# facebookresearch/any4

Hardware: AMD Instinct MI355X
Metric: any4 W4A16 GEMM achieved GB/s (m=1, n=k=4096, g=128) (higher is better)
Workload: dtype bf16

## Files before the change

any4_amd/csrc/tg_gemv.hip:

```cpp
#include "tg_common.cuh"
namespace {
#include "w4_helpers.cuh"
#include "w4_gemv.cuh"

#ifndef TG_GEMV_MF_MIN_M
#define TG_GEMV_MF_MIN_M 1
#endif
#ifndef TG_GEMV_MAX_TILES
#define TG_GEMV_MAX_TILES 16384
#endif
}

#if GEMV_TRACE
static TraceRing g_trace;
extern "C" TG_API void tg_dev_gemv_trace(unsigned long long* buf, int slots) { g_trace.set(buf, slots); }
#endif

int tgx::gemv(const GemmParams& p) {
  const int g0 = 1 << p.gshift;
#ifndef TG_GEMV_MF_MAX_M
#define TG_GEMV_MF_MAX_M 8
#endif
  const bool mf = p.m >= TG_GEMV_MF_MIN_M && p.m <= TG_GEMV_MF_MAX_M && (g0 == 128 || g0 == 256) && (p.k <= 4096 || p.m <= 4) && p.ksuper % 2 == 0;
  if (p.inner != 4 || p.qmx || (p.m > 4 && !mf) || p.x_tc || p.y_tc || p.batch != 1) return TG_PAIR_NA;
  if (p.ksuper * 64 != p.k || p.ntiles * 8 != p.wrows || p.ntiles > TG_GEMV_MAX_TILES) return TG_PAIR_NA;
  const int g = 1 << p.gshift;
  const int gps = g == 32 ? 2 : 1;
  GemvParams gp;
  copy_call(gp, p);
  gp.sg_shift = g <= 64 ? 0 : g == 128 ? 1 : 2;
  gp.trace = nullptr;
  gp.cm = (mf && p.m >= 6 && (p.k == 4096 || p.k == 2048)) ? 1 : 0;
  gp.unit = p.epilogue == TG_EPI_SWIGLU ? 2 : 1;
  if (p.ntiles % gp.unit != 0) return TG_PAIR_NA;
  const int units = p.ntiles / gp.unit;
  const int cus = plan_cu_count(p);
#ifndef TG_GEMV_WG2_MIN_BYTES
#define TG_GEMV_WG2_MIN_BYTES (48ll << 20)
#endif
  auto lds_two_per_cu = [&]() -> int64_t {
    const int tpw2 = ((units + 2 * cus - 1) / (2 * cus)) * gp.unit;
    const int64_t xs = (int64_t)p.m * (p.k / 4), xsmf = mf ? (int64_t)(p.k / 128) * 64 : 0;
    return 65536 + (p.qtype == TG_Q_ANY4_ROWWISE ? tpw2 * 8 * 32 : 0) + (int64_t)p.m * (p.k * 2 + (p.m > 1 ? 16 : 0)) + (xsmf > xs ? xsmf : xs) +
           2 * 8 * p.m * 32 * 4 + 8 * p.m * 4;
  };
  auto padded_tiles = [&](int n_wgs) -> int64_t {
    const int ub = units / n_wgs, ur = units % n_wgs;
    auto pad2 = [&](int u) -> int64_t { return (int64_t)((u * gp.unit + 1) / 2) * 2; };
    return ur * pad2(ub + 1) + (int64_t)(n_wgs - ur) * pad2(ub);
  };
#ifndef TG_GEMV_WG2_MIN_UNITS_PER_CU
#define TG_GEMV_WG2_MIN_UNITS_PER_CU 4
#endif
  const bool two_per_cu = (int64_t)p.wrows * p.k / 2 >= TG_GEMV_WG2_MIN_BYTES && units >= TG_GEMV_WG2_MIN_UNITS_PER_CU * cus && lds_two_per_cu() <= 80 * 1024 &&
                          padded_tiles(2 * cus) <= padded_tiles(cus);
  const int wgs = units < cus ? units : (two_per_cu ? 2 * cus : cus);
  gp.ubase = units / wgs;
  gp.urem = units % wgs;
  gp.uextra = 1;
#ifndef TG_GEMV_WG2_EXTRA
#define TG_GEMV_WG2_EXTRA 3
#endif
  if (TG_GEMV_WG2_EXTRA > 1 && two_per_cu && wgs == 2 * cus && units % cus == 0 && (units / cus) % 2 == 1 && units / cus > TG_GEMV_WG2_EXTRA) {
    gp.ubase = (units / cus - TG_GEMV_WG2_EXTRA) / 2;
    gp.urem = cus;
    gp.uextra = TG_GEMV_WG2_EXTRA;
  }
  gp.uh = 0;
  const int tpw = (gp.ubase + (gp.urem ? gp.uextra : 0)) * gp.unit;
#ifndef TG_GEMV_P_BIG
#define TG_GEMV_P_BIG 16
#endif
  gp.P = mf ? 16 : tpw <= 1 ? 8 : tpw <= 2 ? 16 : TG_GEMV_P_BIG;
  if (p.ksuper % 2 != 0) gp.P = 32;
  else if (p.ksuper % 4 != 0 && gp.P < 16) gp.P = 16;
  gp.p_shift = gp.P == 8 ? 3 : gp.P == 16 ? 4 : 5;
  const int tpp = gp.P / 8;
  const int passes = (tpw + tpp - 1) / tpp;
  const int SS = 32 / gp.P;
  gp.spw = ((p.ksuper + 7) / 8 + SS - 1) / SS * SS;
  gp.spp = gp.spw / SS;
  const int d = gp.spp <= 4 ? 4 : 8;
  gp.rounds = (gp.spp + d - 1) / d;
  gp.xcd4 = (gp.urem == 0 && wgs % 32 == 0) ? 1 : 0;
  if (p.k > 16384) return TG_PAIR_NA;
  gp.lds_lut = 65536;
  const bool stage_lut = p.qtype == TG_Q_ANY4_ROWWISE && passes > 1;
  gp.x_pitch = p.k * 2 + (p.m > 1 ? 16 : 0);
  gp.lds_x = gp.lds_lut + (stage_lut ? tpw * 8 * 32 : 0);
  gp.xs_pitch = p.k / 4;
  gp.lds_xs = gp.lds_x + p.m * gp.x_pitch;
  gp.lds_red = gp.lds_xs + (mf && (p.k / 128) * 64 > p.m * gp.xs_pitch ? (p.k / 128) * 64 : p.m * gp.xs_pitch);
  gp.lds_nrm = gp.lds_red + 2 * 8 * p.m * 32 * 4;
  const unsigned lds = (unsigned)gp.lds_nrm + (unsigned)(8 * p.m * 4);
  if (lds > 160u * 1024u) return TG_PAIR_NA;
  if (p.dry) return TG_PLAN_GEMV;
  const dim3 grid((unsigned)wgs, (unsigned)p.batch);
#if GEMV_TRACE
  gp.trace = g_trace.next();
#endif
  return pick_dt(p.dt, [&](auto DT_) {
    using DT = decltype(DT_);
    return pick<1, 2, 3, 4, 5, 6, 7, 8>(p.m, [&](auto M_) {
      return pick<1, 2>(gps, [&](auto GPS_) {
        return pick<4, 8>(d, [&](auto D_) {
          return pick<0, 1>(p.norm_w != nullptr, [&](auto NORM_) {
            return pick<0, 1>(mf, [&](auto MF_) {
              constexpr int M = decltype(M_)::value, GPS = decltype(GPS_)::value, D = decltype(D_)::value;
              constexpr bool NORM = decltype(NORM_)::value, MF = decltype(MF_)::value;
              if constexpr (MF ? (M < TG_GEMV_MF_MIN_M || GPS != 1 || (D == 8 && M > 4)) : M > 4) {
                return (int)TG_PAIR_NA;
              } else {
                return launch_lds_kernel<w4_gemv_kernel<DT, M, GPS, D, NORM, MF>>(grid, dim3(512), lds, p.st, gp, true);
              }
            });
          });
        });
      });
    });
  });
}
```

any4_amd/csrc/w4_gemv.cuh:

```cuda
#pragma once

struct GemvParams {
  const char* x;
  const char* w;
  const char* qinfo;
  const char* lut;
  char* y;
  const char* bias;
  const char* norm_w;
  int64_t stride_x, stride_w, stride_qinfo, stride_lut, stride_y, stride_bias;
  int64_t bias_row_stride;
  int32_t m, wrows, k;
  int32_t ntiles;
  int32_t ksuper;
  int32_t qtype;
  int32_t sg_shift;
  int32_t P, p_shift;
  int32_t unit;
  int32_t ubase, urem;
  int32_t uextra;
  int32_t uh;
  int32_t spw;
  int32_t spp;
  int32_t rounds;
  int32_t x_pitch, xs_pitch;
  int32_t lds_lut, lds_x, lds_xs, lds_red, lds_nrm;
  float norm_eps;
  int32_t epilogue;
  int32_t xcd4;
  int32_t cm;
  unsigned long long* trace;
};

template <typename DT, int M, int GPS, int D, bool NORM, bool MF = false>
__global__ void __launch_bounds__(512, 2) w4_gemv_kernel(const GemvParams p) {
  static_assert(!MF || GPS == 1, "matrix-core contraction: groups of at least two super-tiles");
#ifndef TG_GEMV_MF_ONES_MIN_M
#define TG_GEMV_MF_ONES_MIN_M 5
#endif
  constexpr bool MFS = MF && M >= TG_GEMV_MF_ONES_MIN_M;
  constexpr int NW = 8, NT = NW * 64;
  const int tid = threadIdx.x;
  const int lane = tid & 63;
  const int wave = __builtin_amdgcn_readfirstlane(tid >> 6);
  constexpr int b = 0;
  TG_TRACE_BEGIN();
  TG_STAMP(0);

  asm volatile("" ::"s"(p.x), "s"(p.w), "s"(p.qinfo), "s"(p.lut), "s"(p.y), "s"(p.bias), "s"(p.norm_w), "s"(p.stride_x), "s"(p.stride_w),
               "s"(p.stride_qinfo), "s"(p.stride_lut), "s"(p.stride_y), "s"(p.stride_bias), "s"(p.bias_row_stride));
  asm volatile("" ::"s"(p.m), "s"(p.wrows), "s"(p.k), "s"(p.ksuper), "s"(p.qtype), "s"(p.sg_shift), "s"(p.P), "s"(p.p_shift), "s"(p.unit),
               "s"(p.ubase), "s"(p.urem), "s"(p.spw), "s"(p.spp), "s"(p.rounds), "s"(p.x_pitch), "s"(p.xs_pitch), "s"(p.lds_lut),
               "s"(p.lds_x), "s"(p.lds_xs), "s"(p.lds_red), "s"(p.lds_nrm), "s"(p.norm_eps), "s"(p.epilogue), "s"(p.xcd4), "s"(p.cm), "s"(p.uextra), "s"(p.uh));
  TG_STAMP(6);

  int bx = blockIdx.x;
  if (p.xcd4) bx = (((bx >> 5) * 8 + (bx & 7)) << 2) + ((bx >> 3) & 3);
  int t0 = bx * p.ubase + min(bx, p.urem) * p.uextra, nu = p.ubase + (bx < p.urem ? p.uextra : 0);
  if (p.uh) {
    const int c = bx < p.urem ? bx : bx - p.urem;
    t0 += bx < p.urem ? min(c, p.uh) : p.uh - min(c, p.uh);
    nu += c < p.uh ? (bx < p.urem ? 1 : -1) : 0;
  }
  t0 *= p.unit;
  const int t1 = t0 + nu * p.unit;
  if (t0 >= t1) return;
  const int P = p.P, Pm = P - 1, tpp = P >> 3;
  const int passes = (t1 - t0 + tpp - 1) >> (p.p_shift - 3);
  const int row_l = lane & Pm;
  const int sub = lane >> p.p_shift;
  const int h = sub & 1, ss = sub >> 1;
  const int SS = 32 >> p.p_shift;
  const int s_begin = wave * p.spw;
  const int s_end = min(s_begin + p.spw, p.ksuper);
  const int spp = p.spp;
  const int rounds = p.rounds;

  const char* wb = p.w + (int64_t)b * p.stride_w;
  const char* qb = p.qinfo + (int64_t)b * p.stride_qinfo;
  const char* lb = p.lut + (int64_t)b * p.stride_lut;
  const char* xb = p.x + (int64_t)b * p.stride_x;

  struct Slot {
    u32x4 w;
    uint32_t q[GPS];
  };
  Slot ring[D];
  int ip = 0, ii = 0;
  uint32_t wlane, qlane;
  const uint32_t qrow_bytes = (uint32_t)p.wrows * 4u;
  auto pass_lane = [&](int pass) {
    const int tile = min(t0 + pass * tpp + (row_l >> 3), t1 - 1);
    wlane = (uint32_t)tile * (uint32_t)p.ksuper * 256u + (uint32_t)((row_l & 7) * 32 + h * 16 + ss * 256);
    qlane = (uint32_t)(tile * 8 + (row_l & 7)) * 4u + (uint32_t)(GPS == 1 ? (ss >> p.sg_shift) : 2 * ss) * qrow_bytes;
  };
  pass_lane(0);
  const int slots = rounds * D;
  const int su_max = p.ksuper - SS;
  auto issue = [&](Slot& sl) {
    const int su = min(s_begin + min(ii, spp - 1) * SS, su_max);
    sl.w = __builtin_nontemporal_load(reinterpret_cast<const u32x4*>(wb + (uint32_t)su * 256u + wlane));
    if constexpr (GPS == 1) {
      sl.q[0] = *reinterpret_cast<const uint32_t*>(qb + (uint32_t)(su >> p.sg_shift) * qrow_bytes + qlane);
    } else {
      sl.q[0] = *reinterpret_cast<const uint32_t*>(qb + (uint32_t)(2 * su) * qrow_bytes + qlane);
      sl.q[1] = *reinterpret_cast<const uint32_t*>(qb + (uint32_t)(2 * su + 1) * qrow_bytes + qlane);
    }
    if (++ii == slots) {
      ii = 0;
      if (ip + 1 < passes) pass_lane(++ip);
      else ii = slots - 1;
    }
  };

  const int npc = p.k >> 3;
  const int nch = p.k >> 5;
  const bool wide = npc > NT;
  uint32_t xd[M][16];
  uint32_t gwd[NORM ? 16 : 1];
  auto stage_load = [&](const char* base, uint32_t (&d)[16]) {
    if (!wide) {
      const int pc = min(tid, npc - 1);
      const char* src = base + (pc >> 2) * 64 + (pc & 3) * 4;
#pragma unroll
      for (int j = 0; j < 4; ++j) d[j] = *reinterpret_cast<const uint32_t*>(src + j * 16);
#pragma unroll
      for (int j = 4; j < 16; ++j) d[j] = 0u;
    } else {
      const u32x4* src = reinterpret_cast<const u32x4*>(base + min(tid, nch - 1) * 64);
#pragma unroll
      for (int j = 0; j < 4; ++j) {
        const u32x4 v = src[j];
        d[4 * j] = v[0]; d[4 * j + 1] = v[1]; d[4 * j + 2] = v[2]; d[4 * j + 3] = v[3];
      }
    }
  };
  bool cm = false;
  int cm_row = 0, cm_chunk = 0, cm_rpr = 1;
  if constexpr (M >= 5) {
    cm = p.cm != 0;
    cm_rpr = NT / nch;
    cm_row = tid / nch;
    cm_chunk = tid - cm_row * nch;
  }
  if (M >= 5 && cm) {
#pragma unroll
    for (int j = 0; j < M; ++j) {
      if (j * cm_rpr < M) {
        const int row = min(j * cm_rpr + cm_row, M - 1);
        const u32x4* src = reinterpret_cast<const u32x4*>(xb + (int64_t)row * p.k * 2 + cm_chunk * 64);
#pragma unroll
        for (int q = 0; q < 4; ++q) {
          const u32x4 v = src[q];
          xd[j][4 * q] = v[0]; xd[j][4 * q + 1] = v[1]; xd[j][4 * q + 2] = v[2]; xd[j][4 * q + 3] = v[3];
        }
      }
    }
    if constexpr (NORM) {
      const u32x4* src = reinterpret_cast<const u32x4*>(p.norm_w + cm_chunk * 64);
#pragma unroll
      for (int q = 0; q < 4; ++q) {
        const u32x4 v = src[q];
        gwd[4 * q] = v[0]; gwd[4 * q + 1] = v[1]; gwd[4 * q + 2] = v[2]; gwd[4 * q + 3] = v[3];
      }
    }
  } else {
#pragma unroll
  for (int a = 0; a < M; ++a) stage_load(xb + (int64_t)a * p.k * 2, xd[a]);
  if constexpr (NORM) stage_load(p.norm_w, gwd);
  }
  const int c = tid & 31;
  const int hi = tid >> 5;
  uint32_t lp[8];
  const bool rowwise = p.qtype == TG_Q_ANY4_ROWWISE;
  const int wg_rows = (t1 - t0) * 8;
  if (p.qtype == TG_Q_INT4) {
#pragma unroll
    for (int e = 0; e < 16; e += 2) lp[e >> 1] = DT::pack2((float)(e - 8), (float)(e - 7));
  } else {
    const int trow = min(t0 + ((c & Pm) >> 3), t1 - 1) * 8 + (c & 7);
    const char* lsrc = lb + (rowwise ? (int64_t)trow * 32 : 0);
    const u32x4 l0 = reinterpret_cast<const u32x4*>(lsrc)[0];
    const u32x4 l1 = reinterpret_cast<const u32x4*>(lsrc)[1];
#pragma unroll
    for (int j = 0; j < 4; ++j) { lp[j] = l0[j]; lp[4 + j] = l1[j]; }
  }
  const bool stage_lut = rowwise && passes > 1;
  u32x4 lstage = {0, 0, 0, 0};
  if (stage_lut) lstage = reinterpret_cast<const u32x4*>(lb + (int64_t)t0 * 256)[min(tid, wg_rows * 2 - 1)];
  uint16_t res0 = 0;
  if (p.bias) {
    const int a = min(tid >> p.p_shift, M - 1), r = tid & Pm;
    const int row = min(t0 + (r >> 3), t1 - 1) * 8 + (r & 7);
    res0 = *reinterpret_cast<const uint16_t*>(p.bias + (int64_t)b * p.stride_bias + ((int64_t)a * p.bias_row_stride + row) * 2);
  }
  asm volatile("s_barrier" ::: "memory");
#pragma unroll
  for (int j = 0; j < D; ++j) {
    __builtin_amdgcn_sched_barrier(0);
    issue(ring[j]);
  }
  __builtin_amdgcn_sched_barrier(0);
  TG_STAMP(1);
  const uint32_t lds_x = (uint32_t)p.lds_x, lds_xs = (uint32_t)p.lds_xs, lds_red = (uint32_t)p.lds_red;
  auto piece_store = [&](int a, int pc, uint32_t d0, uint32_t d1, uint32_t d2, uint32_t d3, bool on) -> float {
    u32x4 o;
    o[0] = __builtin_amdgcn_perm(d1, d0, 0x05040100u);
    o[1] = __builtin_amdgcn_perm(d3, d2, 0x05040100u);
    o[2] = __builtin_amdgcn_perm(d1, d0, 0x07060302u);
    o[3] = __builtin_amdgcn_perm(d3, d2, 0x07060302u);
    float sum = 0.f;
#pragma unroll
    for (int j = 0; j < 4; ++j) sum = dot2_ones<DT>(o[j], sum);
    if (on) *(lds_u32x4ptr)(lds_x + (uint32_t)(a * p.x_pitch + pc * 16)) = o;
    return sum;
  };
  auto xs_store = [&](int a, int ch, int hh, float sum) {
    *(lds_fptr)(lds_xs + (uint32_t)(a * p.xs_pitch + (((ch >> 1) * 2 + hh) * 2 + (ch & 1)) * 4)) = sum;
  };
  if (M >= 5 && cm) {
    float nrm[M];
#pragma unroll
    for (int a = 0; a < M; ++a) nrm[a] = 0.f;
#pragma unroll
    for (int j = 0; j < M; ++j) {
      if (j * cm_rpr < M) {
        const int a = j * cm_rpr + cm_row;
        const bool on = a < M;
        if constexpr (NORM) {
          float v = 0.f;
#pragma unroll
          for (int e = 0; e < 16; ++e) {
            if constexpr (std::is_same<DT, BF16>::value)
              v = __builtin_amdgcn_fdot2_f32_bf16(__builtin_bit_cast(bf16x2, xd[j][e]), __builtin_bit_cast(bf16x2, xd[j][e]), v, false);
            else
              v = __builtin_amdgcn_fdot2(__builtin_bit_cast(f16x2, xd[j][e]), __builtin_bit_cast(f16x2, xd[j][e]), v, false);
          }
          v = on ? v : 0.f;
          v = tgl::wave_sum(v);
#pragma unroll
          for (int a2 = 0; a2 < M; ++a2) nrm[a2] = a2 == a ? v : nrm[a2];
#pragma unroll
          for (int e = 0; e < 16; ++e) {
            const uint32_t xv = xd[j][e], g = gwd[e];
            xd[j][e] = DT::pack2(DT::lo_f32(xv) * DT::lo_f32(g), DT::hi_f32(xv) * DT::hi_f32(g));
          }
        }
        float sum = 0.f;
#pragma unroll
        for (int q = 0; q < 4; ++q) sum += piece_store(on ? a : 0, 4 * cm_chunk + q, xd[j][q], xd[j][q + 4], xd[j][q + 8], xd[j][q + 12], on);
        if constexpr (!MFS) {
          sum = on ? sum : 0.f;
          sum += tgl::lane_xor<1>(sum, lane);
          sum += tgl::lane_xor<2>(sum, lane);
          if (on && (cm_chunk & 3) == 0) *(lds_fptr)(lds_xs + (uint32_t)((cm_chunk >> 2) * 64 + a * 4)) = sum;
        }
      }
    }
    if constexpr (NORM) {
      if (lane == 0) {
#pragma unroll
        for (int a = 0; a < M; ++a) *(lds_fptr)((uint32_t)p.lds_nrm + (uint32_t)((wave * M + a) * 4)) = nrm[a];
      }
    }
  } else {
#pragma unroll
  for (int a = 0; a < M; ++a) {
    const bool on = wide ? tid < nch : tid < npc;
    if constexpr (NORM) {
      float v = 0.f;
#pragma unroll
      for (int j = 0; j < 16; ++j) {
        if constexpr (std::is_same<DT, BF16>::value)
          v = __builtin_amdgcn_fdot2_f32_bf16(__builtin_bit_cast(bf16x2, xd[a][j]), __builtin_bit_cast(bf16x2, xd[a][j]), v, false);
        else
          v = __builtin_amdgcn_fdot2(__builtin_bit_cast(f16x2, xd[a][j]), __builtin_bit_cast(f16x2, xd[a][j]), v, false);
      }
      v = on ? v : 0.f;
      v = tgl::wave_sum(v);
      if (lane == 0) *(lds_fptr)((uint32_t)p.lds_nrm + (uint32_t)((wave * M + a) * 4)) = v;
#pragma unroll
      for (int j = 0; j < 16; ++j) {
        const uint32_t xv = xd[a][j], g = gwd[j];
        xd[a][j] = DT::pack2(DT::lo_f32(xv) * DT::lo_f32(g), DT::hi_f32(xv) * DT::hi_f32(g));
      }
    }
    if (MF && M <= 4 && wide) {
      float sum = 0.f;
#pragma unroll
      for (int q = 0; q < 4; ++q) sum += piece_store(a, 4 * tid + q, xd[a][q], xd[a][q + 4], xd[a][q + 8], xd[a][q + 12], on);
      if constexpr (!MFS) {
        sum = on ? sum : 0.f;
        sum += tgl::lane_xor<1>(sum, lane);
        sum += tgl::lane_xor<2>(sum, lane);
        if (on && (tid & 3) == 0) *(lds_fptr)(lds_xs + (uint32_t)((tid >> 2) * 64 + a * 4)) = sum;
      }
    } else if (MF) {
      float sum = piece_store(a, tid, xd[a][0], xd[a][1], xd[a][2], xd[a][3], on);
      if constexpr (!MFS) {
        sum = on ? sum : 0.f;
        sum = tgl::row_sum(sum);
        if (on && (tid & 15) == 0) *(lds_fptr)(lds_xs + (uint32_t)((tid >> 4) * 64 + a * 4)) = sum;
      }
    } else if (!wide) {
      float sum = piece_store(a, tid, xd[a][0], xd[a][1], xd[a][2], xd[a][3], on);
      sum += tgl::lane_xor<1>(sum, lane);
      if (on && (tid & 1) == 0) xs_store(a, tid >> 2, (tid >> 1) & 1, sum);
    } else {
      float sq[4];
#pragma unroll
      for (int q = 0; q < 4; ++q) sq[q] = piece_store(a, 4 * tid + q, xd[a][q], xd[a][q + 4], xd[a][q + 8], xd[a][q + 12], on);
      if (on) {
        xs_store(a, tid, 0, sq[0] + sq[1]);
        xs_store(a, tid, 1, sq[2] + sq[3]);
      }
    }
  }
  }
  if (stage_lut && tid < wg_rows * 2) *(lds_u32x4ptr)((uint32_t)p.lds_lut + (uint32_t)tid * 16u) = lstage;
  if (stage_lut)
    for (int i = tid + NT; i < wg_rows * 2; i += NT)
      *(lds_u32x4ptr)((uint32_t)p.lds_lut + (uint32_t)i * 16u) = reinterpret_cast<const u32x4*>(lb + (int64_t)t0 * 256)[i];

  auto build_table = [&](int half) {
    uint32_t hsel = lp[0];
#pragma unroll
    for (int j = 1; j < 8; ++j) hsel = (hi >> 1) == j ? lp[j] : hsel;
    const uint32_t hv = (hi & 1) ? (hsel & 0xffff0000u) : (hsel << 16);
    const lds_u32ptr tb = (lds_u32ptr)((uint32_t)(hi * 16 * 256 + (half * 32 + c) * 4));
#pragma unroll
    for (int lo = 0; lo < 16; ++lo) {
      const uint32_t lv = (lo & 1) ? (lp[lo >> 1] >> 16) : (lp[lo >> 1] & 0xffffu);
      tb[lo * 64] = lv | hv;
    }
  };
  build_table(0);
  TG_STAMP(2);
  __syncthreads();
  TG_STAMP(3);

  uint32_t colreg = (uint32_t)((lane & 31) * 4);
  float yacc[MF ? 4 : M];
#pragma unroll
  for (int a = 0; a < (MF ? 4 : M); ++a) yacc[a] = 0.f;

  auto pass_end = [&](int cp) {
    const uint32_t par = (uint32_t)(cp & 1);
    if constexpr (MF) {
#pragma unroll
      for (int r = 0; r < 4; ++r) {
        const int a = 4 * (lane >> 4) + r;
        if (a < M) *(lds_fptr)(lds_red + (uint32_t)((((par * NW + wave) * M + a) * 32 + (lane & 15)) * 4)) = yacc[r];
        yacc[r] = 0.f;
      }
    } else {
    float v[M];
#pragma unroll
    for (int a = 0; a < M; ++a) {
      v[a] = yacc[a];
      yacc[a] = 0.f;
      v[a] = tgl::halves32_sum(v[a]);
      if (P <= 16) v[a] = tgl::rows16_sum(v[a]);
      if (P <= 8) v[a] += tgl::lane_xor<8>(v[a], lane);
    }
    if (lane < P) {
#pragma unroll
      for (int a = 0; a < M; ++a) *(lds_fptr)(lds_red + (uint32_t)((((par * NW + wave) * M + a) * 32 + lane) * 4)) = v[a];
    }
    }
    if (rowwise && cp + 1 < passes) {
      const int lrow = min((cp + 1) * P + (c & Pm), wg_rows - 1);
      const u32x4 l0 = *(lds_cu32x4ptr)((uint32_t)p.lds_lut + (uint32_t)lrow * 32u);
      const u32x4 l1 = *(lds_cu32x4ptr)((uint32_t)p.lds_lut + (uint32_t)lrow * 32u + 16u);
#pragma unroll
      for (int j = 0; j < 4; ++j) { lp[j] = l0[j]; lp[4 + j] = l1[j]; }
      build_table((cp + 1) & 1);
      colreg ^= 128u;
    }
    __syncthreads();
    if (tid < P * M) {
      const int a = tid >> p.p_shift, r = tid & Pm;
      const int tile = t0 + cp * tpp + (r >> 3);
      if (tile < t1) {
        const int row = tile * 8 + (r & 7);
        float sum = 0.f;
#pragma unroll
        for (int w8 = 0; w8 < NW; ++w8) sum += *(lds_fptr)(lds_red + (uint32_t)((((par * NW + w8) * M + a) * 32 + r) * 4));
        float rsn = 1.f;
        if constexpr (NORM) {
          float tot = 0.f;
#pragma unroll
          for (int w8 = 0; w8 < NW; ++w8) tot += *(lds_fptr)((uint32_t)p.lds_nrm + (uint32_t)((w8 * M + a) * 4));
          rsn = rsqrtf(tot * (1.0f / (float)p.k) + p.norm_eps);
          sum *= rsn;
        }
        if (p.epilogue == TG_EPI_SWIGLU) {
          if ((r & 15) < 8) {
            float up = 0.f;
#pragma unroll
            for (int w8 = 0; w8 < NW; ++w8) up += *(lds_fptr)(lds_red + (uint32_t)((((par * NW + w8) * M + a) * 32 + r + 8) * 4));
            up *= rsn;
            if constexpr (NORM && !std::is_same<DT, BF16>::value) asm volatile("" : "+v"(up));
            *reinterpret_cast<uint16_t*>(p.y + (int64_t)b * p.stride_y + ((int64_t)a * (p.wrows >> 1) + ((row >> 4) << 3) + (row & 7)) * 2) = swiglu16<DT>(sum, up);
          }
        } else {
          uint16_t o16 = DT::from_f32(sum);
          if (p.bias) {
            uint16_t bv = res0;
            if (cp > 0) bv = *reinterpret_cast<const uint16_t*>(p.bias + (int64_t)b * p.stride_bias + ((int64_t)a * p.bias_row_stride + row) * 2);
            o16 = DT::from_f32(DT::lo_f32(o16) + DT::lo_f32(bv));
          }
          *reinterpret_cast<uint16_t*>(p.y + (int64_t)b * p.stride_y + ((int64_t)a * p.wrows + row) * 2) = o16;
        }
      }
    }
  };

  const uint32_t xlane = lds_x + (uint32_t)(ss * 128 + h * 32), xslane = lds_xs + (uint32_t)((ss * 2 + h) * 8);
  auto consume = [&](const Slot& sl, int i) {
    const int su_l = s_begin + i * SS;
    const bool on = su_l < s_end;
    const int su = min(su_l, su_max);
    const uint32_t xa = xlane + (uint32_t)su * 128u;
    const uint32_t xsa = xslane + (uint32_t)su * 16u;
    if constexpr (MF) {
      const uint32_t xr = xa + (uint32_t)(min(lane & 15, M - 1) * p.x_pitch);
      f32x4 acc = {0.f, 0.f, 0.f, 0.f};
      u32x4 e4[4], xf4[4];
#pragma unroll
      for (int u = 0; u < 4; ++u) {
        const int jc = u >> 1, qq = u & 1;
        const uint32_t w = sl.w[qq * 2 + jc];
#pragma unroll
        for (int j = 0; j < 4; ++j) e4[u][j] = *(lds_cu32ptr)(__builtin_amdgcn_perm(w, colreg, 0x0c0c0400u + ((uint32_t)j << 8)));
        xf4[u] = *(lds_cu32x4ptr)(xr + (uint32_t)(jc * 64 + qq * 16));
      }
      f32x4 gs4 = {0.f, 0.f, 0.f, 0.f};
      if constexpr (!MFS) {
        const f32x4 v = *(lds_cf32x4ptr)(lds_xs + (uint32_t)((su >> 1) * 64 + (lane >> 4) * 16));
        gs4 = f32x4{v[0], v[1], v[2], v[3]};
      }
      __builtin_amdgcn_sched_barrier(0);
#pragma unroll
      for (int u = 0; u < 4; ++u) acc = DT::mfma(xf4[u], e4[u], acc);
      if constexpr (MFS) {
        const uint32_t one2 = DT::pack2(1.f, 1.f);
        const u32x4 ones = {one2, one2, one2, one2};
#pragma unroll
        for (int u = 0; u < 4; ++u) gs4 = DT::mfma(xf4[u], ones, gs4);
      }
      const float sc = on ? DT::lo_f32(sl.q[0]) : 0.f;
      const float zz = on ? DT::hi_f32(sl.q[0]) : 0.f;
#pragma unroll
      for (int r = 0; r < 4; ++r) yacc[r] = __builtin_fmaf(zz, gs4[r], __builtin_fmaf(sc, acc[r], yacc[r]));
      return;
    }
    float dsum[M][GPS];
#pragma unroll
    for (int a = 0; a < M; ++a)
#pragma unroll
      for (int g = 0; g < GPS; ++g) dsum[a][g] = 0.f;
    uint32_t e[4][4];
    u32x4 xf[M][4];
#pragma unroll
    for (int u = 0; u < 4; ++u) {
      const int jc = u >> 1, qq = u & 1;
      const uint32_t w = sl.w[qq * 2 + jc];
#pragma unroll
      for (int j = 0; j < 4; ++j) e[u][j] = *(lds_cu32ptr)(__builtin_amdgcn_perm(w, colreg, 0x0c0c0400u + ((uint32_t)j << 8)));
#pragma unroll
      for (int a = 0; a < M; ++a) xf[a][u] = *(lds_cu32x4ptr)(xa + (uint32_t)(a * p.x_pitch + jc * 64 + qq * 16));
    }
    __builtin_amdgcn_sched_barrier(0);
#pragma unroll
    for (int u = 0; u < 4; ++u) {
      const int jc = u >> 1;
#pragma unroll
      for (int a = 0; a < M; ++a)
#pragma unroll
        for (int j = 0; j < 4; ++j) dsum[a][GPS == 1 ? 0 : jc] = dot2<DT>(e[u][j], xf[a][u][j], dsum[a][GPS == 1 ? 0 : jc]);
    }
#pragma unroll
    for (int g = 0; g < GPS; ++g) {
      const float sc = on ? DT::lo_f32(sl.q[g]) : 0.f;
      const float zz = on ? DT::hi_f32(sl.q[g]) : 0.f;
#pragma unroll
      for (int a = 0; a < M; ++a) {
        const f32x2 xs2 = *(const __attribute__((address_space(3))) f32x2*)(xsa + (uint32_t)(a * p.xs_pitch));
        const float xs = GPS == 1 ? xs2[0] + xs2[1] : xs2[g];
        yacc[a] = __builtin_fmaf(zz, xs, __builtin_fmaf(sc, dsum[a][g], yacc[a]));
      }
    }
  };

  for (int cp = 0; cp < passes; ++cp) {
    const bool last = cp + 1 == passes;
    const int nr = rounds - (last ? 1 : 0);
    for (int r = 0; r < nr; ++r) {
#pragma unroll
      for (int j = 0; j < D; ++j) {
        if (r * D + j < spp) consume(ring[j], r * D + j);
        issue(ring[j]);
        TG_STAMP_IF(cp == 0 && r == 0 && j == 0, 4);
      }
    }
    if (last) {
#pragma unroll
      for (int j = 0; j < D; ++j) {
        if ((rounds - 1) * D + j < spp) consume(ring[j], (rounds - 1) * D + j);
        TG_STAMP_IF(cp == 0 && rounds == 1 && j == 0, 4);
      }
    }
    pass_end(cp);
  }
  TG_STAMP(5);
  TG_TRACE_FLUSH(tid == 0 && p.trace, p.trace, 7);
}
```

Before: 6603.

## Run GEMV load ring continuously across passes instead of draining per pass

Replaces the per-pass ring of depth 4 or 8 (rounded up to whole rounds, with padded slots and a drain at each pass end) with a continuous depth-4 ring that spans all passes. Loads for the next pass are issued while the current pass is still being consumed, and pass_end runs at block boundaries inside the loop. The ring kind is chosen on the host from total steps and spp divisibility. The aim is to remove the pipeline drain and refill bubbles between passes and the wasted padded loads. The cost is a shallower prefetch depth (4 instead of 8 for larger spp) and more control logic inside the unrolled loop.

```diff
diff --git a/any4_amd/csrc/gemv_ring.h b/any4_amd/csrc/gemv_ring.h
--- /dev/null
+++ b/any4_amd/csrc/gemv_ring.h
@@ -0,0 +1,60 @@
+#pragma once
+#include <stdint.h>
+
+#if defined(__HIPCC__)
+#define TG_RING_FN __host__ __device__ __forceinline__
+#else
+#define TG_RING_FN inline
+#endif
+
+struct GemvRingKind {
+  int32_t D, B;
+};
+enum { GEMV_RING_KINDS = 2 };
+TG_RING_FN constexpr GemvRingKind gemv_ring_kind(int i) { return i == 0 ? GemvRingKind{4, 4} : GemvRingKind{4, 1}; }
+
+TG_RING_FN int gemv_ring_choose(int total_min, int spp, unsigned mask) {
+  for (int i = 0; i + 1 < GEMV_RING_KINDS; ++i) {
+    const GemvRingKind k = gemv_ring_kind(i);
+    if (((mask >> i) & 1u) && k.D <= total_min && spp % k.B == 0) return i;
+  }
+  return GEMV_RING_KINDS - 1;
+}
+
+TG_RING_FN int gemv_ring_rounds(int total, int D) { return total / D; }
+TG_RING_FN int gemv_ring_tail(int total, int D) { return total % D; }
+
+TG_RING_FN int gemv_ring_first(int total, int j) { return j < total ? j : total - 1; }
+
+TG_RING_FN int gemv_ring_refill(int total, int D, int i) { return i + D < total ? i + D : -1; }
+
+struct GemvRingStep {
+  int32_t pass, step;
+  int32_t slot;
+  int32_t refill;
+  int32_t ends_pass;
+};
+
+TG_RING_FN GemvRingStep gemv_ring_step(int spp, int passes, int D, int i) {
+  GemvRingStep s;
+  s.pass = i / spp;
+  s.step = i - s.pass * spp;
+  s.slot = i % D;
+  s.refill = gemv_ring_refill(spp * passes, D, i);
+  s.ends_pass = s.step + 1 == spp;
+  return s;
+}
+
+struct GemvRingCursor {
+  int32_t pass, step;
+};
+TG_RING_FN bool gemv_ring_advance(GemvRingCursor& c, int spp, int passes) {
+  if (++c.step < spp) return false;
+  if (c.pass + 1 < passes) {
+    ++c.pass;
+    c.step = 0;
+    return true;
+  }
+  c.step = spp - 1;
+  return false;
+}
diff --git a/any4_amd/csrc/tg_gemv.hip b/any4_amd/csrc/tg_gemv.hip
--- a/any4_amd/csrc/tg_gemv.hip
+++ b/any4_amd/csrc/tg_gemv.hip
@@ -1,4 +1,5 @@
 #include "tg_common.cuh"
+#include "gemv_ring.h"
 namespace {
 #include "w4_helpers.cuh"
 #include "w4_gemv.cuh"
@@ -80,8 +81,8 @@
   const int SS = 32 / gp.P;
   gp.spw = ((p.ksuper + 7) / 8 + SS - 1) / SS * SS;
   gp.spp = gp.spw / SS;
-  const int d = gp.spp <= 4 ? 4 : 8;
-  gp.rounds = (gp.spp + d - 1) / d;
+  const int tiles_min = gp.ubase > 0 ? gp.ubase * gp.unit : tpw;
+  const int kind = gemv_ring_choose(((tiles_min + tpp - 1) / tpp) * gp.spp, gp.spp, (1u << GEMV_RING_KINDS) - 1u);
   gp.xcd4 = (gp.urem == 0 && wgs % 32 == 0) ? 1 : 0;
   if (p.k > 16384) return TG_PAIR_NA;
   gp.lds_lut = 65536;
@@ -103,15 +104,16 @@
     using DT = decltype(DT_);
     return pick<1, 2, 3, 4, 5, 6, 7, 8>(p.m, [&](auto M_) {
       return pick<1, 2>(gps, [&](auto GPS_) {
-        return pick<4, 8>(d, [&](auto D_) {
+        return pick<0, 1>(kind, [&](auto K_) {
           return pick<0, 1>(p.norm_w != nullptr, [&](auto NORM_) {
             return pick<0, 1>(mf, [&](auto MF_) {
-              constexpr int M = decltype(M_)::value, GPS = decltype(GPS_)::value, D = decltype(D_)::value;
+              constexpr int M = decltype(M_)::value, GPS = decltype(GPS_)::value;
+              constexpr int D = gemv_ring_kind(decltype(K_)::value).D, B = gemv_ring_kind(decltype(K_)::value).B;
               constexpr bool NORM = decltype(NORM_)::value, MF = decltype(MF_)::value;
-              if constexpr (MF ? (M < TG_GEMV_MF_MIN_M || GPS != 1 || (D == 8 && M > 4)) : M > 4) {
+              if constexpr (MF ? (M < TG_GEMV_MF_MIN_M || GPS != 1) : M > 4) {
                 return (int)TG_PAIR_NA;
               } else {
-                return launch_lds_kernel<w4_gemv_kernel<DT, M, GPS, D, NORM, MF>>(grid, dim3(512), lds, p.st, gp, true);
+                return launch_lds_kernel<w4_gemv_kernel<DT, M, GPS, D, B, NORM, MF>>(grid, dim3(512), lds, p.st, gp, true);
               }
             });
           });
diff --git a/any4_amd/csrc/w4_gemv.cuh b/any4_amd/csrc/w4_gemv.cuh
--- a/any4_amd/csrc/w4_gemv.cuh
+++ b/any4_amd/csrc/w4_gemv.cuh
@@ -22,7 +22,6 @@
   int32_t uh;
   int32_t spw;
   int32_t spp;
-  int32_t rounds;
   int32_t x_pitch, xs_pitch;
   int32_t lds_lut, lds_x, lds_xs, lds_red, lds_nrm;
   float norm_eps;
@@ -32,7 +31,17 @@
   unsigned long long* trace;
 };
 
-template <typename DT, int M, int GPS, int D, bool NORM, bool MF = false>
+template <int D, int B, int T = 0, typename F>
+__device__ __forceinline__ void gemv_tail_pick(int t, F&& f) {
+  if constexpr (T + B >= D) {
+    f(std::integral_constant<int, T>{});
+  } else {
+    if (t == T) f(std::integral_constant<int, T>{});
+    else gemv_tail_pick<D, B, T + B>(t, f);
+  }
+}
+
+template <typename DT, int M, int GPS, int D, int B, bool NORM, bool MF = false>
 __global__ void __launch_bounds__(512, 2) w4_gemv_kernel(const GemvParams p) {
   static_assert(!MF || GPS == 1, "matrix-core contraction: groups of at least two super-tiles");
 #ifndef TG_GEMV_MF_ONES_MIN_M
@@ -50,7 +59,7 @@
   asm volatile("" ::"s"(p.x), "s"(p.w), "s"(p.qinfo), "s"(p.lut), "s"(p.y), "s"(p.bias), "s"(p.norm_w), "s"(p.stride_x), "s"(p.stride_w),
                "s"(p.stride_qinfo), "s"(p.stride_lut), "s"(p.stride_y), "s"(p.stride_bias), "s"(p.bias_row_stride));
   asm volatile("" ::"s"(p.m), "s"(p.wrows), "s"(p.k), "s"(p.ksuper), "s"(p.qtype), "s"(p.sg_shift), "s"(p.P), "s"(p.p_shift), "s"(p.unit),
-               "s"(p.ubase), "s"(p.urem), "s"(p.spw), "s"(p.spp), "s"(p.rounds), "s"(p.x_pitch), "s"(p.xs_pitch), "s"(p.lds_lut),
+               "s"(p.ubase), "s"(p.urem), "s"(p.spw), "s"(p.spp), "s"(p.x_pitch), "s"(p.xs_pitch), "s"(p.lds_lut),
                "s"(p.lds_x), "s"(p.lds_xs), "s"(p.lds_red), "s"(p.lds_nrm), "s"(p.norm_eps), "s"(p.epilogue), "s"(p.xcd4), "s"(p.cm), "s"(p.uextra), "s"(p.uh));
   TG_STAMP(6);
 
@@ -74,7 +83,7 @@
   const int s_begin = wave * p.spw;
   const int s_end = min(s_begin + p.spw, p.ksuper);
   const int spp = p.spp;
-  const int rounds = p.rounds;
+  const int total = passes * spp;
 
   const char* wb = p.w + (int64_t)b * p.stride_w;
   const char* qb = p.qinfo + (int64_t)b * p.stride_qinfo;
@@ -86,7 +95,7 @@
     uint32_t q[GPS];
   };
   Slot ring[D];
-  int ip = 0, ii = 0;
+  GemvRingCursor rq = {0, 0};
   uint32_t wlane, qlane;
   const uint32_t qrow_bytes = (uint32_t)p.wrows * 4u;
   auto pass_lane = [&](int pass) {
@@ -95,10 +104,9 @@
     qlane = (uint32_t)(tile * 8 + (row_l & 7)) * 4u + (uint32_t)(GPS == 1 ? (ss >> p.sg_shift) : 2 * ss) * qrow_bytes;
   };
   pass_lane(0);
-  const int slots = rounds * D;
   const int su_max = p.ksuper - SS;
   auto issue = [&](Slot& sl) {
-    const int su = min(s_begin + min(ii, spp - 1) * SS, su_max);
+    const int su = min(s_begin + rq.step * SS, su_max);
     sl.w = __builtin_nontemporal_load(reinterpret_cast<const u32x4*>(wb + (uint32_t)su * 256u + wlane));
     if constexpr (GPS == 1) {
       sl.q[0] = *reinterpret_cast<const uint32_t*>(qb + (uint32_t)(su >> p.sg_shift) * qrow_bytes + qlane);
@@ -106,11 +114,7 @@
       sl.q[0] = *reinterpret_cast<const uint32_t*>(qb + (uint32_t)(2 * su) * qrow_bytes + qlane);
       sl.q[1] = *reinterpret_cast<const uint32_t*>(qb + (uint32_t)(2 * su + 1) * qrow_bytes + qlane);
     }
-    if (++ii == slots) {
-      ii = 0;
-      if (ip + 1 < passes) pass_lane(++ip);
-      else ii = slots - 1;
-    }
+    if (gemv_ring_advance(rq, spp, passes)) pass_lane(rq.pass);
   };
 
   const int npc = p.k >> 3;
@@ -493,26 +497,45 @@
     }
   };
 
-  for (int cp = 0; cp < passes; ++cp) {
-    const bool last = cp + 1 == passes;
-    const int nr = rounds - (last ? 1 : 0);
-    for (int r = 0; r < nr; ++r) {
+  const int q = gemv_ring_rounds(total, D), t = gemv_ring_tail(total, D);
+  int cp = 0, ci = 0;
+  auto boundary = [&]() {
+    if (ci == spp) {
+      pass_end(cp);
+      ++cp;
+      ci = 0;
+    }
+  };
+  for (int r = 0; r + 1 < q; ++r) {
+#pragma unroll
+    for (int j = 0; j < D; ++j) {
+      if (ci < spp) consume(ring[j], ci);
+      ++ci;
+      issue(ring[j]);
+      TG_STAMP_IF(r == 0 && j == 0, 4);
+      if ((j + 1) % B == 0) boundary();
+    }
+  }
+  auto tail = [&](auto T_) {
+    constexpr int T = decltype(T_)::value;
+    if (q > 0) {
 #pragma unroll
       for (int j = 0; j < D; ++j) {
-        if (r * D + j < spp) consume(ring[j], r * D + j);
-        issue(ring[j]);
-        TG_STAMP_IF(cp == 0 && r == 0 && j == 0, 4);
-      }
-    }
-    if (last) {
-#pragma unroll
-      for (int j = 0; j < D; ++j) {
-        if ((rounds - 1) * D + j < spp) consume(ring[j], (rounds - 1) * D + j);
-        TG_STAMP_IF(cp == 0 && rounds == 1 && j == 0, 4);
-      }
-    }
-    pass_end(cp);
-  }
+        if (ci < spp) consume(ring[j], ci);
+        ++ci;
+        if (j < T) issue(ring[j]);
+        TG_STAMP_IF(q == 1 && j == 0, 4);
+        if ((j + 1) % B == 0) boundary();
+      }
+    }
+#pragma unroll
+    for (int j = 0; j < T; ++j) {
+      if (ci < spp) consume(ring[j], ci);
+      ++ci;
+      if ((j + 1) % B == 0) boundary();
+    }
+  };
+  gemv_tail_pick<D, B>(t, tail);
   TG_STAMP(5);
   TG_TRACE_FLUSH(tid == 0 && p.trace, p.trace, 7);
 }
```

Result: no change. 6605, median of 2 (+0.0%).
